# tingyu215/VACNIC

Hardware: AMD Instinct MI355X
Metric: train samples/sec, BART-large + CLIP ViT-L/14 full VACNIC step, GoodNews-shaped batch (higher is better)
Workload: dtype bf16

## Files before the change

### vacnic_amd/csrc/attn.hip

```cpp
#include "common.h"

namespace {

constexpr float FMIN = -3.4028234663852886e38f;
constexpr int OOB = 0x7ffffff0;
constexpr int TILE_B = 64 * 64 * 2;

__device__ __forceinline__ int swz(int row) { return (((row >> 1) & 1) << 2) | ((row >> 2) & 3); }

__device__ __forceinline__ void stage64(__amdgpu_buffer_rsrc_t rsrc, char* tile, int row0, int nrows, int ld,
                                        int wave, int lane) {
#pragma unroll
  for (int i = 0; i < 2; ++i) {
    const int blk = wave * 2 + i;
    const int row = blk * 8 + (lane >> 3);
    const int lc = (lane & 7) ^ swz(row);
    const int gr = row0 + row;
    const int voff = gr < nrows ? (int)(((unsigned)gr * (unsigned)ld + (unsigned)(lc * 8)) * 2u) : OOB;
    __builtin_amdgcn_raw_ptr_buffer_load_lds(rsrc, LDS_PTR(tile + blk * 1024), 16, voff, 0, 0, 0);
  }
}

__device__ __forceinline__ bf16x8 frag_row(const char* tile, int rbase, int ks, int lane) {
  const int row = rbase + (lane & 31);
  const int chunk = 2 * ks + (lane >> 5);
  return *(const bf16x8*)(tile + row * 128 + ((chunk ^ swz(row)) << 4));
}
__device__ __forceinline__ bf16x8 frag_tr(const char* tile, int rbase, int cbase, int lane) {
  const int g = lane >> 4, i = lane & 15, h = lane >> 5;
  const int col = cbase + 16 * (g & 1) + 4 * (i & 3);
  bf16x8 r;
#pragma unroll
  for (int hh = 0; hh < 2; ++hh) {
    const int row = rbase + 8 * hh + 4 * h + (i >> 2);
    const char* a = tile + row * 128 + (((col >> 3) ^ swz(row)) << 4) + (col & 7) * 2;
    bf16x4 t = __builtin_amdgcn_ds_read_tr16_b64_v4i16((__attribute__((address_space(3))) bf16x4*)LDS_PTR(a));
    r[4 * hh + 0] = t[0]; r[4 * hh + 1] = t[1]; r[4 * hh + 2] = t[2]; r[4 * hh + 3] = t[3];
  }
  return r;
}
__device__ __forceinline__ bf16x8 pack_acc(const f32x16& x, int s) {
  bf16x8 r;
#pragma unroll
  for (int j = 0; j < 8; ++j) r[j] = (short)f2bf(x[8 * s + j]);
  return r;
}
__device__ __forceinline__ bf16x8 gload8(__amdgpu_buffer_rsrc_t rsrc, int voff) {
  u32x4 v = __builtin_amdgcn_raw_buffer_load_b128(rsrc, voff, 0, 0);
  return *(bf16x8*)&v;
}
__device__ __forceinline__ int acc_row(int r, int h) { return (r & 3) + 8 * (r >> 2) + 4 * h; }

__device__ __forceinline__ void lds_barrier() {
  asm volatile("s_waitcnt lgkmcnt(0)" ::: "memory");
  __builtin_amdgcn_s_barrier();
}

struct AttnP {
  const bf16_t* q; const bf16_t* k; const bf16_t* v; bf16_t* out; float* lse;
  const bf16_t* dout; const float* delta; float* delta_out; bf16_t* dq; bf16_t* dk; bf16_t* dv;
  const uint8_t* key_mask;
  int B, H, Tq, Tk;
  int ldq, ldk, ldv, ldo, lddq, lddk, lddv;
  long bsq, bsk, bsv, bso, bsdq, bsdk, bsdv;
  int causal; float scale;
  unsigned drop_thr; float drop_inv; unsigned long long drop_seed; const unsigned long long* drop_seed_dev;
};

struct DropCtx { unsigned long long seed; unsigned long long bh_base; unsigned pk_per_row; unsigned thr; float inv; };

__device__ __forceinline__ DropCtx drop_ctx(const AttnP& p, int b, int hd) {
  DropCtx d;
  d.seed = p.drop_seed_dev ? p.drop_seed ^ (*p.drop_seed_dev * 0x9E3779B97F4A7C15ull) : p.drop_seed;
  d.pk_per_row = (unsigned)((p.Tk + 3) >> 2);
  d.bh_base = ((unsigned long long)b * p.H + hd) * (unsigned long long)((p.Tq + 3) >> 2) * d.pk_per_row;
  d.thr = p.drop_thr; d.inv = p.drop_inv;
  return d;
}
__device__ __forceinline__ void drop_patch(const DropCtx& d, int q, int k, uint32_t w[4]) {
  const unsigned long long idx = d.bh_base + (unsigned long long)(q >> 2) * d.pk_per_row + (unsigned)(k >> 2);
  philox4x32((uint32_t)idx, (uint32_t)(idx >> 32), 0x41545444u, 0u, (uint32_t)d.seed, (uint32_t)(d.seed >> 32), w);
}
#define VAC_QUAD_BCAST(V_, G_) ((uint32_t)__builtin_amdgcn_update_dpp(0, (int)(V_), (G_) * 0x55, 0xf, 0xf, true))
__device__ __forceinline__ void drop_block_keys(const DropCtx& d, int q, int kblock, int lane, uint32_t mw[4]) {
  const int i = lane & 3;
  uint32_t w[4];
  drop_patch(d, q, kblock + 8 * i, w);
#define VAC_TAKE(G_)                                                                                   \
  {                                                                                                    \
    const uint32_t t0 = VAC_QUAD_BCAST(w[0], G_), t1 = VAC_QUAD_BCAST(w[1], G_);                       \
    const uint32_t t2 = VAC_QUAD_BCAST(w[2], G_), t3 = VAC_QUAD_BCAST(w[3], G_);                       \
    mw[G_] = i == 0 ? t0 : i == 1 ? t1 : i == 2 ? t2 : t3;                                             \
  }
  VAC_TAKE(0) VAC_TAKE(1) VAC_TAKE(2) VAC_TAKE(3)
#undef VAC_TAKE
}
__device__ __forceinline__ void drop_word_factors(const DropCtx& d, uint32_t x, float m[4]) {
#pragma unroll
  for (int e = 0; e < 4; ++e) m[e] = ((x >> (8 * e)) & 0xffu) >= d.thr ? d.inv : 0.f;
}
__device__ __forceinline__ void drop_block_queries(const DropCtx& d, int qblock, int k, int lane, uint32_t mb[4]) {
  const int i = lane & 3, sh = 8 * i;
  uint32_t w[4];
  drop_patch(d, qblock + 8 * i, k, w);
#define VAC_TAKE(G_)                                                                                   \
  {                                                                                                    \
    const uint32_t t0 = VAC_QUAD_BCAST(w[0], G_), t1 = VAC_QUAD_BCAST(w[1], G_);                       \
    const uint32_t t2 = VAC_QUAD_BCAST(w[2], G_), t3 = VAC_QUAD_BCAST(w[3], G_);                       \
    mb[G_] = ((t0 >> sh) & 0xffu) | (((t1 >> sh) & 0xffu) << 8) | (((t2 >> sh) & 0xffu) << 16) | (((t3 >> sh) & 0xffu) << 24); \
  }
  VAC_TAKE(0) VAC_TAKE(1) VAC_TAKE(2) VAC_TAKE(3)
#undef VAC_TAKE
}

__device__ __forceinline__ __amdgpu_buffer_rsrc_t make_rsrc(const bf16_t* base, int rows, int ld) {
  const unsigned bytes = rows > 0 ? ((unsigned)(rows - 1) * (unsigned)ld + 64u) * 2u : 0u;
  return __builtin_amdgcn_make_buffer_rsrc((void*)base, 0, bytes, 0x00020000);
}

__device__ __forceinline__ void fill_key_bias(float* kbias, unsigned* dirty, const uint8_t* mask_row, int Tk, int Tk_pad) {
  for (int j = threadIdx.x; j < Tk_pad; j += 256) {
    float b = 0.f;
    if (j >= Tk) b = -INFINITY;
    else if (mask_row && mask_row[j] == 0) b = FMIN;
    kbias[j] = b;
    const unsigned long long any = __builtin_amdgcn_ballot_w64(b != 0.f);
    if ((threadIdx.x & 63) == 0) dirty[j >> 6] = any != 0ull;
  }
}


__device__ __forceinline__ void xcd_order(int nblk, int H, int nbh, int& blk, int& hd, int& b) {
  const int L = blockIdx.x;
  int bh;
  if ((nbh & 7) == 0) { const int x = L & 7, j = L >> 3; bh = x + 8 * (j / nblk); blk = j % nblk; }
  else { bh = L / nblk; blk = L % nblk; }
  b = bh / H; hd = bh - b * H;
}

template <bool CAUSAL, bool DROP>
__global__ __launch_bounds__(256, 2) void attn_fwd_kernel(AttnP p) {
  extern __shared__ __attribute__((aligned(16))) char smem[];
  const int tid = threadIdx.x, lane = tid & 63;
  const int wave = __builtin_amdgcn_readfirstlane(tid >> 6);
  int b, hd, qblk;
  xcd_order((p.Tq + 127) >> 7, p.H, p.B * p.H, qblk, hd, b);
  const int q0 = qblk * 128 + wave * 32;
  const int ql = lane & 31, hh = lane >> 5;
  const int Tk_pad = (p.Tk + 63) & ~63;
// ... 72 lines not shown
        }
      m_run = m_new;
    } else {
#pragma unroll
      for (int kb2 = 0; kb2 < 2; ++kb2) {
#pragma unroll
        for (int g = 0; g < 4; ++g) {
          const int kbase = t * 64 + kb2 * 32 + 8 * g + 4 * hh;
          const f32x4 bias = *(const f32x4*)(kbias + kbase);
#pragma unroll
          for (int e = 0; e < 4; ++e) {
            float v = fmaf(s[kb2][4 * g + e], scale2, bias[e]);
            if (CAUSAL && (kbase + e) > qidx) v += FMIN;
            s[kb2][4 * g + e] = v;
            tmax = fmaxf(tmax, v);
          }
        }
      }
      tmax = fmaxf(tmax, __shfl_xor(tmax, 32, 64));
      const float m_new = fmaxf(m_run, tmax);
      alpha = __builtin_amdgcn_exp2f(m_run - m_new);
#pragma unroll
      for (int kb2 = 0; kb2 < 2; ++kb2)
#pragma unroll
        for (int r = 0; r < 16; ++r) {
          const float e = __builtin_amdgcn_exp2f(s[kb2][r] - m_new);
          s[kb2][r] = e;
          psum += e;
        }
      m_run = m_new;
    }
    l_run = l_run * alpha + psum;
    if (DROP) {
#pragma unroll
      for (int kb2 = 0; kb2 < 2; ++kb2) {
        uint32_t mw[4];
        drop_block_keys(dctx, qidx, t * 64 + kb2 * 32 + 4 * hh, lane, mw);
#pragma unroll
        for (int g = 0; g < 4; ++g) {
          float mk[4];
          drop_word_factors(dctx, mw[g], mk);
#pragma unroll
          for (int e = 0; e < 4; ++e) s[kb2][4 * g + e] *= mk[e];
        }
      }
    }
#pragma unroll
    for (int r = 0; r < 16; ++r) { o[0][r] *= alpha; o[1][r] *= alpha; }
#pragma unroll
    for (int kb2 = 0; kb2 < 2; ++kb2)
#pragma unroll
      for (int ss = 0; ss < 2; ++ss) {
        const bf16x8 pf = pack_acc(s[kb2], ss);
#pragma unroll
        for (int hb = 0; hb < 2; ++hb)
          o[hb] = __builtin_amdgcn_mfma_f32_32x32x16_bf16(frag_tr(vt, kb2 * 32 + 16 * ss, hb * 32, lane), pf, o[hb], 0, 0, 0);
      }
    lds_barrier();
  }

  const float l_tot = l_run + __shfl_xor(l_run, 32, 64);
  const float inv = 1.f / l_tot;
  {
    char* ot = smem + wave * 4096;
#pragma unroll
    for (int hb = 0; hb < 2; ++hb)
#pragma unroll
      for (int g = 0; g < 4; ++g) {
        const u32x2 pk = {pack2bf(o[hb][4 * g] * inv, o[hb][4 * g + 1] * inv),
                          pack2bf(o[hb][4 * g + 2] * inv, o[hb][4 * g + 3] * inv)};
        const int c16 = hb * 4 + g;
        *(u32x2*)(ot + ql * 128 + ((c16 ^ (ql & 7)) << 4) + 8 * hh) = pk;
      }
    asm volatile("s_waitcnt lgkmcnt(0)" ::: "memory");
#pragma unroll
    for (int i = 0; i < 4; ++i) {
      const int row = (lane >> 3) + 8 * i, c16 = lane & 7;
      const int qrow = q0 + row;
      const u32x4 v = *(const u32x4*)(ot + row * 128 + ((c16 ^ (row & 7)) << 4));
      if (qrow < p.Tq) *(u32x4*)(p.out + (long)b * p.bso + (long)qrow * p.ldo + hd * 64 + c16 * 8) = v;
    }
  }
  if (qidx < p.Tq && p.lse && hh == 0) p.lse[((long)b * p.H + hd) * p.Tq + qidx] = m_run * 0.6931471805599453f + __logf(l_tot);
}

__global__ __launch_bounds__(256) void attn_delta_kernel(const bf16_t* __restrict__ o, const bf16_t* __restrict__ dout,
                                                         float* __restrict__ delta, int B, int H, int Tq, int ldo,
                                                         long bso) {
  const int lane = threadIdx.x & 63;
  const long row = (long)blockIdx.x * 4 + (threadIdx.x >> 6);
  if (row >= (long)B * Tq) return;
  const int b = (int)(row / Tq), q = (int)(row % Tq);
  const bf16_t* orow = o + (long)b * bso + (long)q * ldo;
  const bf16_t* drow = dout + (long)b * bso + (long)q * ldo;
  for (int c = lane; c < H * 8; c += 64) {
    u32x4 a = *(const u32x4*)(orow + c * 8), d = *(const u32x4*)(drow + c * 8);
    float s = 0.f;
#pragma unroll
    for (int i = 0; i < 4; ++i) {
      s += __uint_as_float(a[i] << 16) * __uint_as_float(d[i] << 16);
      s += __uint_as_float(a[i] & 0xffff0000u) * __uint_as_float(d[i] & 0xffff0000u);
    }
    s += __shfl_xor(s, 1, 64); s += __shfl_xor(s, 2, 64); s += __shfl_xor(s, 4, 64);
    if ((c & 7) == 0) delta[((long)b * H + (c >> 3)) * Tq + q] = s;
  }
}

template <bool DROP>
__global__ __launch_bounds__(256, 2) void attn_bwd_dkv_kernel(AttnP p) {
  extern __shared__ __attribute__((aligned(16))) char smem[];
  const int tid = threadIdx.x, lane = tid & 63;
  const int wave = __builtin_amdgcn_readfirstlane(tid >> 6);
  int b, hd, kblk;
  xcd_order((p.Tk + 127) >> 7, p.H, p.B * p.H, kblk, hd, b);
  const int k0 = kblk * 128 + wave * 32;
  const int kl = lane & 31, hh = lane >> 5;
  const int kidx = k0 + kl;
  float* stats = (float*)(smem + 4 * TILE_B);
  constexpr float LOG2E = 1.4426950408889634f;
  const float scale2 = p.scale * LOG2E;

  const bf16_t* qb = p.q + (long)b * p.bsq + hd * 64;
  const bf16_t* kb = p.k + (long)b * p.bsk + hd * 64;
  const bf16_t* vb = p.v + (long)b * p.bsv + hd * 64;
  const bf16_t* dob = p.dout + (long)b * p.bso + hd * 64;
  __amdgpu_buffer_rsrc_t qs = make_rsrc(qb, p.Tq, p.ldq);
  __amdgpu_buffer_rsrc_t ks = make_rsrc(kb, p.Tk, p.ldk);
  __amdgpu_buffer_rsrc_t vs = make_rsrc(vb, p.Tk, p.ldv);
  __amdgpu_buffer_rsrc_t dos = make_rsrc(dob, p.Tq, p.ldo);
  const float* lse = p.lse + ((long)b * p.H + hd) * p.Tq;
  const float* delta = p.delta + ((long)b * p.H + hd) * p.Tq;

  const int nq_tiles = (p.Tq + 63) >> 6;
  int t_begin = 0;
  if (p.causal) t_begin = min(nq_tiles, (kblk * 128) >> 6);

  bf16x8 kf[4], vf[4];
#pragma unroll
  for (int s = 0; s < 4; ++s) {
    kf[s] = gload8(ks, kidx < p.Tk ? (int)(((unsigned)kidx * (unsigned)p.ldk + 16u * s + 8u * hh) * 2u) : OOB);
    vf[s] = gload8(vs, kidx < p.Tk ? (int)(((unsigned)kidx * (unsigned)p.ldv + 16u * s + 8u * hh) * 2u) : OOB);
  }
  float kbias = 0.f;
  if (kidx >= p.Tk) kbias = -INFINITY;
  else if (p.key_mask && p.key_mask[(long)b * p.Tk + kidx] == 0) kbias = FMIN;

  f32x16 dk[2], dv[2];
  dk[0] = (f32x16)(0.f); dk[1] = (f32x16)(0.f); dv[0] = (f32x16)(0.f); dv[1] = (f32x16)(0.f);
  DropCtx dctx;
  if (DROP) dctx = drop_ctx(p, b, hd);

  auto load_stat = [&](int t) -> float {
    float v = 0.f;
    if (tid < 128) {
      const int qi = t * 64 + (tid & 63);
      if (tid < 64) v = qi < p.Tq ? lse[qi] : INFINITY;
      else v = qi < p.Tq ? delta[qi] : 0.f;
    }
    return v;
  };
  auto put_stat = [&](float* st, float sv) {
    if (tid < 128) st[tid] = sv;
    if (tid < 64) st[128 + tid] = -sv * LOG2E;
  };
  const bool plain = !p.causal && __builtin_amdgcn_ballot_w64(kbias != 0.f) == 0ull;

  if (t_begin < nq_tiles) {
    const float sv = load_stat(t_begin);
    stage64(qs, smem, t_begin * 64, p.Tq, p.ldq, wave, lane);
    stage64(dos, smem + TILE_B, t_begin * 64, p.Tq, p.ldo, wave, lane);
    put_stat(stats, sv);
  }
  for (int t = t_begin; t < nq_tiles; ++t) {
    const int cur = (t - t_begin) & 1;
    char* qt = smem + cur * (2 * TILE_B);
    char* dot = qt + TILE_B;
    if (t + 1 < nq_tiles) {
      char* nq = smem + (cur ^ 1) * (2 * TILE_B);
      const float sv = load_stat(t + 1);
      stage64(qs, nq, (t + 1) * 64, p.Tq, p.ldq, wave, lane);
      stage64(dos, nq + TILE_B, (t + 1) * 64, p.Tq, p.ldo, wave, lane);
      put_stat(stats + (cur ^ 1) * 192, sv);
      asm volatile("s_waitcnt vmcnt(4)" ::: "memory");
    } else {
      asm volatile("s_waitcnt vmcnt(0)" ::: "memory");
    }
    lds_barrier();
    const float* st = stats + cur * 192;

#pragma unroll
    for (int qb2 = 0; qb2 < 2; ++qb2) {
      f32x16 s = (f32x16)(0.f), dp = (f32x16)(0.f);
#pragma unroll
      for (int ks4 = 0; ks4 < 4; ++ks4) {
        s = __builtin_amdgcn_mfma_f32_32x32x16_bf16(frag_row(qt, qb2 * 32, ks4, lane), kf[ks4], s, 0, 0, 0);
        dp = __builtin_amdgcn_mfma_f32_32x32x16_bf16(frag_row(dot, qb2 * 32, ks4, lane), vf[ks4], dp, 0, 0, 0);
      }
      uint32_t mb[4];
      if (DROP) drop_block_queries(dctx, t * 64 + qb2 * 32 + 4 * hh, kidx, lane, mb);
#pragma unroll
      for (int g = 0; g < 4; ++g) {
        const int ql0 = qb2 * 32 + 8 * g + 4 * hh;
        const f32x4 l4 = *(const f32x4*)(st + ql0);
        const f32x4 d4 = *(const f32x4*)(st + 64 + ql0);
        float mq[4] = {1.f, 1.f, 1.f, 1.f};
        if (DROP) drop_word_factors(dctx, mb[g], mq);
        if (plain) {
          const f32x4 nl4 = *(const f32x4*)(st + 128 + ql0);
#pragma unroll
          for (int e = 0; e < 4; ++e) {
            const float pe = __builtin_amdgcn_exp2f(fmaf(s[4 * g + e], scale2, nl4[e]));
            s[4 * g + e] = DROP ? pe * mq[e] : pe;
            dp[4 * g + e] = pe * ((DROP ? dp[4 * g + e] * mq[e] : dp[4 * g + e]) - d4[e]);
          }
        } else {
#pragma unroll
          for (int e = 0; e < 4; ++e) {
            float v = s[4 * g + e] * p.scale + kbias;
            if (p.causal && kidx > (t * 64 + ql0 + e)) v += FMIN;
            const float pe = __expf(v - l4[e]);
            s[4 * g + e] = DROP ? pe * mq[e] : pe;
            dp[4 * g + e] = pe * ((DROP ? dp[4 * g + e] * mq[e] : dp[4 * g + e]) - d4[e]);
          }
        }
      }
#pragma unroll
      for (int ss = 0; ss < 2; ++ss) {
        const bf16x8 pf = pack_acc(s, ss), dsf = pack_acc(dp, ss);
#pragma unroll
        for (int hb = 0; hb < 2; ++hb) {
          dv[hb] = __builtin_amdgcn_mfma_f32_32x32x16_bf16(frag_tr(dot, qb2 * 32 + 16 * ss, hb * 32, lane), pf, dv[hb], 0, 0, 0);
          dk[hb] = __builtin_amdgcn_mfma_f32_32x32x16_bf16(frag_tr(qt, qb2 * 32 + 16 * ss, hb * 32, lane), dsf, dk[hb], 0, 0, 0);
        }
      }
    }
    lds_barrier();
  }

  if (kidx < p.Tk) {
    bf16_t* dkrow = p.dk + (long)b * p.bsdk + (long)kidx * p.lddk + hd * 64;
    bf16_t* dvrow = p.dv + (long)b * p.bsdv + (long)kidx * p.lddv + hd * 64;
#pragma unroll
    for (int hb = 0; hb < 2; ++hb)
#pragma unroll
      for (int g = 0; g < 4; ++g) {
        u32x2 a = {pack2bf(dk[hb][4 * g] * p.scale, dk[hb][4 * g + 1] * p.scale), pack2bf(dk[hb][4 * g + 2] * p.scale, dk[hb][4 * g + 3] * p.scale)};
        u32x2 c = {pack2bf(dv[hb][4 * g], dv[hb][4 * g + 1]), pack2bf(dv[hb][4 * g + 2], dv[hb][4 * g + 3])};
        *(u32x2*)(dkrow + hb * 32 + 8 * g + 4 * hh) = a;
        *(u32x2*)(dvrow + hb * 32 + 8 * g + 4 * hh) = c;
      }
  }
}

template <bool DROP, bool DELTA_PASS>
__global__ __launch_bounds__(256, 2) void attn_bwd_dq_kernel(AttnP p) {
  extern __shared__ __attribute__((aligned(16))) char smem[];
  const int tid = threadIdx.x, lane = tid & 63;
  const int wave = __builtin_amdgcn_readfirstlane(tid >> 6);
  int b, hd, qblk;
  xcd_order((p.Tq + 127) >> 7, p.H, p.B * p.H, qblk, hd, b);
  const int q0 = qblk * 128 + wave * 32;
  const int ql = lane & 31, hh = lane >> 5;
  const int qidx = q0 + ql;
  const int Tk_pad = (p.Tk + 63) & ~63;
  float* kbias = (float*)(smem + 4 * TILE_B);
  unsigned* dirty = (unsigned*)(kbias + Tk_pad);
  constexpr float LOG2E = 1.4426950408889634f;
  const float scale2 = p.scale * LOG2E;

  const bf16_t* qb = p.q + (long)b * p.bsq + hd * 64;
  const bf16_t* kb = p.k + (long)b * p.bsk + hd * 64;
  const bf16_t* vb = p.v + (long)b * p.bsv + hd * 64;
  const bf16_t* dob = p.dout + (long)b * p.bso + hd * 64;
  __amdgpu_buffer_rsrc_t qs = make_rsrc(qb, p.Tq, p.ldq);
  __amdgpu_buffer_rsrc_t ks = make_rsrc(kb, p.Tk, p.ldk);
  __amdgpu_buffer_rsrc_t vs = make_rsrc(vb, p.Tk, p.ldv);
  __amdgpu_buffer_rsrc_t dos = make_rsrc(dob, p.Tq, p.ldo);

  int ntile = Tk_pad >> 6;
  if (p.causal) ntile = min(ntile, (min(p.Tq, qblk * 128 + 128) + 63) >> 6);

  stage64(ks, smem, 0, p.Tk, p.ldk, wave, lane);
  stage64(vs, smem + TILE_B, 0, p.Tk, p.ldv, wave, lane);
  fill_key_bias(kbias, dirty, p.key_mask ? p.key_mask + (long)b * p.Tk : nullptr, p.Tk, Tk_pad);

  bf16x8 qf[4], dof[4];
#pragma unroll
  for (int s = 0; s < 4; ++s) {
    qf[s] = gload8(qs, qidx < p.Tq ? (int)(((unsigned)qidx * (unsigned)p.ldq + 16u * s + 8u * hh) * 2u) : OOB);
    dof[s] = gload8(dos, qidx < p.Tq ? (int)(((unsigned)qidx * (unsigned)p.ldo + 16u * s + 8u * hh) * 2u) : OOB);
  }
  float lse_q = INFINITY, delta_q = 0.f;
  if (qidx < p.Tq) {
    lse_q = p.lse[((long)b * p.H + hd) * p.Tq + qidx];
    if (!DELTA_PASS) delta_q = p.delta[((long)b * p.H + hd) * p.Tq + qidx];
  }
  const float nl2 = -lse_q * LOG2E;
  float dsum = 0.f;
  f32x16 dq[2];
  dq[0] = (f32x16)(0.f); dq[1] = (f32x16)(0.f);
  DropCtx dctx;
  if (DROP) dctx = drop_ctx(p, b, hd);

  for (int t = 0; t < ntile; ++t) {
    const int cur = t & 1;
    char* kt = smem + cur * (2 * TILE_B);
    char* vt = kt + TILE_B;
    if (t + 1 < ntile) {
      char* nk = smem + (cur ^ 1) * (2 * TILE_B);
      stage64(ks, nk, (t + 1) * 64, p.Tk, p.ldk, wave, lane);
      stage64(vs, nk + TILE_B, (t + 1) * 64, p.Tk, p.ldv, wave, lane);
      asm volatile("s_waitcnt vmcnt(4)" ::: "memory");
    } else {
      asm volatile("s_waitcnt vmcnt(0)" ::: "memory");
    }
    lds_barrier();
    const bool plain = !p.causal && __builtin_amdgcn_readfirstlane((int)dirty[t]) == 0;
#pragma unroll
    for (int kb2 = 0; kb2 < 2; ++kb2) {
      f32x16 s = (f32x16)(0.f), dp = (f32x16)(0.f);
#pragma unroll
      for (int ks4 = 0; ks4 < 4; ++ks4) {
        s = __builtin_amdgcn_mfma_f32_32x32x16_bf16(frag_row(kt, kb2 * 32, ks4, lane), qf[ks4], s, 0, 0, 0);
        dp = __builtin_amdgcn_mfma_f32_32x32x16_bf16(frag_row(vt, kb2 * 32, ks4, lane), dof[ks4], dp, 0, 0, 0);
      }
      uint32_t mw[4];
      if (DROP) drop_block_keys(dctx, qidx, t * 64 + kb2 * 32 + 4 * hh, lane, mw);
#pragma unroll
      for (int g = 0; g < 4; ++g) {
        const int kbase = t * 64 + kb2 * 32 + 8 * g + 4 * hh;
        float mk[4] = {1.f, 1.f, 1.f, 1.f};
        if (DROP) drop_word_factors(dctx, mw[g], mk);
        if (plain) {
#pragma unroll
          for (int e = 0; e < 4; ++e) {
            const float pe = __builtin_amdgcn_exp2f(fmaf(s[4 * g + e], scale2, nl2));
            const float dpm = DROP ? dp[4 * g + e] * mk[e] : dp[4 * g + e];
            if (DELTA_PASS) dsum += pe * dpm;
            else dp[4 * g + e] = pe * (dpm - delta_q);
          }
        } else {
          const f32x4 bias = *(const f32x4*)(kbias + kbase);
#pragma unroll
          for (int e = 0; e < 4; ++e) {
            float v = s[4 * g + e] * p.scale + bias[e];
            if (p.causal && (kbase + e) > qidx) v += FMIN;
            const float pe = __expf(v - lse_q);
            const float dpm = DROP ? dp[4 * g + e] * mk[e] : dp[4 * g + e];
            if (DELTA_PASS) dsum += pe * dpm;
            else dp[4 * g + e] = pe * (dpm - delta_q);
          }
        }
      }
      if (!DELTA_PASS) {
#pragma unroll
        for (int ss = 0; ss < 2; ++ss) {
          const bf16x8 dsf = pack_acc(dp, ss);
#pragma unroll
          for (int hb = 0; hb < 2; ++hb)
            dq[hb] = __builtin_amdgcn_mfma_f32_32x32x16_bf16(frag_tr(kt, kb2 * 32 + 16 * ss, hb * 32, lane), dsf, dq[hb], 0, 0, 0);
        }
      }
    }
    lds_barrier();
  }
  if (DELTA_PASS) {
    dsum += __shfl_xor(dsum, 32, 64);
    if (qidx < p.Tq && hh == 0) p.delta_out[((long)b * p.H + hd) * p.Tq + qidx] = dsum;
    return;
  }
  if (qidx < p.Tq) {
    bf16_t* drow = p.dq + (long)b * p.bsdq + (long)qidx * p.lddq + hd * 64;
#pragma unroll
    for (int hb = 0; hb < 2; ++hb)
#pragma unroll
      for (int g = 0; g < 4; ++g) {
        u32x2 a = {pack2bf(dq[hb][4 * g] * p.scale, dq[hb][4 * g + 1] * p.scale), pack2bf(dq[hb][4 * g + 2] * p.scale, dq[hb][4 * g + 3] * p.scale)};
        *(u32x2*)(drow + hb * 32 + 8 * g + 4 * hh) = a;
      }
  }
}

int set_dropout(AttnP& p, float p_drop, uint64_t seed, const uint64_t* seed_dev, const char* who) {
  if (!(p_drop >= 0.f && p_drop < 1.f)) { vacnic_set_error("%s: p_drop must be in [0, 1)", who); return VACNIC_BAD_SHAPE; }
  unsigned thr = (unsigned)(p_drop * 256.f + 0.5f);
  if (thr > 255) thr = 255;
  p.drop_thr = thr;
  p.drop_inv = 256.f / (256.f - (float)thr);
  p.drop_seed = seed; p.drop_seed_dev = (const unsigned long long*)seed_dev;
  return VACNIC_OK;
}

int check_common(int64_t B, int64_t H, int64_t Tq, int64_t Tk, int64_t ldq, int64_t ldk, int64_t ldv, int64_t ldo,
                 const char* who) {
  if (B <= 0 || H <= 0 || Tq <= 0 || Tk <= 0) {
    vacnic_set_error("%s: empty problem B=%ld H=%ld Tq=%ld Tk=%ld", who, (long)B, (long)H, (long)Tq, (long)Tk);
    return VACNIC_BAD_SHAPE;
  }
  if ((ldq & 7) || (ldk & 7) || (ldv & 7) || (ldo & 7)) {
    vacnic_set_error("%s: row strides must be multiples of 8 elements", who);
    return VACNIC_MISALIGNED;
  }
  if (Tk > 8192 || H > 65535 || B > 65535) {
    vacnic_set_error("%s: Tk=%ld / H / B beyond supported range", who, (long)Tk);
    return VACNIC_UNSUPPORTED;
  }
  return VACNIC_OK;
}

}


template <int NWV>
__global__ __launch_bounds__(64 * NWV) void attn_decode_kernel(AttnP p) {
  extern __shared__ float probs[];
  const int lane = threadIdx.x & 63, h = blockIdx.x, b = blockIdx.y;
  const int wv = NWV == 1 ? 0 : __builtin_amdgcn_readfirstlane(threadIdx.x >> 6);
  const int per = (p.Tk + NWV - 1) / NWV;
  const int k_lo = wv * per, k_hi = min(p.Tk, k_lo + per);
  const bf16_t* q = p.q + (long)b * p.bsq + h * 64;
  const bf16_t* kb = p.k + (long)b * p.bsk + h * 64;
  const bf16_t* vb = p.v + (long)b * p.bsv + h * 64;
  const uint8_t* km = p.key_mask ? p.key_mask + (long)b * p.Tk : nullptr;
  float qf[64];
#pragma unroll
  for (int c = 0; c < 8; ++c) {
    const u32x4 r = *(const u32x4*)(q + c * 8);
#pragma unroll
    for (int i = 0; i < 4; ++i) { qf[c * 8 + 2 * i] = __uint_as_float(r[i] << 16); qf[c * 8 + 2 * i + 1] = __uint_as_float(r[i] & 0xffff0000u); }
  }
  float m = -INFINITY;
  for (int key0 = k_lo + lane; key0 < k_hi; key0 += 256) {
    u32x4 kr[4][8];
#pragma unroll
    for (int u = 0; u < 4; ++u) {
      const int key = key0 + 64 * u;
      const bf16_t* krow = kb + (long)(key < k_hi ? key : key0) * p.ldk;
#pragma unroll
      for (int c = 0; c < 8; ++c) kr[u][c] = *(const u32x4*)(krow + c * 8);
    }
#pragma unroll
    for (int u = 0; u < 4; ++u) {
      const int key = key0 + 64 * u;
      if (key < k_hi) {
        float dot = 0.f;
#pragma unroll
        for (int c = 0; c < 8; ++c)
#pragma unroll
          for (int i = 0; i < 4; ++i) {
            dot += qf[c * 8 + 2 * i] * __uint_as_float(kr[u][c][i] << 16);
            dot += qf[c * 8 + 2 * i + 1] * __uint_as_float(kr[u][c][i] & 0xffff0000u);
          }
        float sc = dot * p.scale;
        if (km && km[key] == 0) sc += -3.4028234663852886e38f;
        probs[key] = sc;
        m = fmaxf(m, sc);
      }
    }
  }
  m = wave_max(m);
  float l = 0.f;
  for (int key = k_lo + lane; key < k_hi; key += 64) {
// ... 38 lines not shown
    }
    if (lane == 0) { pm[wv] = m; pl[wv] = l; }
    __syncthreads();
    if (wv != 0) return;
    float gm = pm[0];
#pragma unroll
    for (int w = 1; w < NWV; ++w) gm = fmaxf(gm, pm[w]);
    float gl = 0.f;
#pragma unroll
    for (int j = 0; j < 8; ++j) acc[j] = 0.f;
#pragma unroll
    for (int w = 0; w < NWV; ++w) {
      const float sc = pl[w] > 0.f ? __expf(pm[w] - gm) : 0.f;
      gl += pl[w] * sc;
      if (kg == 0) {
#pragma unroll
        for (int j = 0; j < 8; ++j) acc[j] += pacc[w * 64 + dc * 8 + j] * sc;
      }
    }
    m = gm; l = gl;
  }
  if (kg == 0) {
    const float inv = 1.f / l;
    bf16_t* o = p.out + (long)b * p.bso + h * 64 + dc * 8;
    *(u32x4*)o = (u32x4){pack2bf(acc[0] * inv, acc[1] * inv), pack2bf(acc[2] * inv, acc[3] * inv),
                         pack2bf(acc[4] * inv, acc[5] * inv), pack2bf(acc[6] * inv, acc[7] * inv)};
  }
  if (p.lse && lane == 0) p.lse[((long)b * p.H + h)] = m + logf(l);
}

extern "C" int vacnic_attn_fwd(const vacnic_attn_fwd_args* a, void* stream) {
  VPLAN_REC_STRUCT(vacnic_attn_fwd, a, stream);
  VCHECK(a && a->q && a->k && a->v && a->out, VACNIC_BAD_SHAPE, "attn_fwd: null operand");
  if (int e = check_common(a->B, a->H, a->Tq, a->Tk, a->ldq, a->ldk, a->ldv, a->ldo, "attn_fwd")) return e;
  VCHECK(aligned16(a->q) && aligned16(a->k) && aligned16(a->v) && aligned16(a->out) && !(a->bsq & 7) && !(a->bsk & 7) &&
         !(a->bsv & 7) && !(a->bso & 7), VACNIC_MISALIGNED, "attn_fwd: pointers/batch strides must be 16-byte aligned");
  AttnP p = {};
  p.q = (const bf16_t*)a->q; p.k = (const bf16_t*)a->k; p.v = (const bf16_t*)a->v; p.out = (bf16_t*)a->out;
  p.lse = a->lse; p.key_mask = a->key_mask;
  p.B = (int)a->B; p.H = (int)a->H; p.Tq = (int)a->Tq; p.Tk = (int)a->Tk;
  p.ldq = (int)a->ldq; p.ldk = (int)a->ldk; p.ldv = (int)a->ldv; p.ldo = (int)a->ldo;
  p.bsq = a->bsq; p.bsk = a->bsk; p.bsv = a->bsv; p.bso = a->bso;
  p.causal = a->causal; p.scale = a->scale;
  if (int e = set_dropout(p, a->p_drop, a->seed, a->seed_dev, "attn_fwd")) return e;
  if (p.Tq == 1 && !p.causal && p.Tk <= 16384 && !p.drop_thr) {
    if (p.Tk >= 256) hipLaunchKernelGGL(attn_decode_kernel<4>, dim3(p.H, p.B), dim3(256), (size_t)(p.Tk + 4 * 64 + 8) * 4, (hipStream_t)stream, p);
    else hipLaunchKernelGGL(attn_decode_kernel<1>, dim3(p.H, p.B), dim3(64), (size_t)p.Tk * 4, (hipStream_t)stream, p);
    VLAUNCH_CHECK();
    return VACNIC_OK;
  }
  const int Tk_pad = (p.Tk + 63) & ~63;
  dim3 grid((unsigned)(((p.Tq + 127) / 128) * p.H * p.B));
  const size_t lds = 4 * TILE_B + Tk_pad * 4 + (Tk_pad >> 6) * 4;
  hipStream_t st = (hipStream_t)stream;
  if (p.drop_thr) {
    if (p.causal) hipLaunchKernelGGL((attn_fwd_kernel<true, true>), grid, dim3(256), lds, st, p);
    else hipLaunchKernelGGL((attn_fwd_kernel<false, true>), grid, dim3(256), lds, st, p);
  } else {
    if (p.causal) hipLaunchKernelGGL((attn_fwd_kernel<true, false>), grid, dim3(256), lds, st, p);
    else hipLaunchKernelGGL((attn_fwd_kernel<false, false>), grid, dim3(256), lds, st, p);
  }
  VLAUNCH_CHECK();
  return VACNIC_OK;
}

extern "C" int vacnic_attn_bwd(const vacnic_attn_bwd_args* a, void* stream) {
  VPLAN_REC_STRUCT(vacnic_attn_bwd, a, stream);
  VCHECK(a && a->q && a->k && a->v && a->out && a->dout && a->lse && a->delta && a->dq && a->dk && a->dv,
         VACNIC_BAD_SHAPE, "attn_bwd: null operand");
  if (int e = check_common(a->B, a->H, a->Tq, a->Tk, a->ldq, a->ldk, a->ldv, a->ldo, "attn_bwd")) return e;
  VCHECK(!(a->lddq & 7) && !(a->lddk & 7) && !(a->lddv & 7) && !(a->bsq & 7) && !(a->bsk & 7) && !(a->bsv & 7) &&
         !(a->bso & 7) && !(a->bsdq & 7) && !(a->bsdk & 7) && !(a->bsdv & 7), VACNIC_MISALIGNED,
         "attn_bwd: strides must be multiples of 8 elements");
  AttnP p = {};
  p.q = (const bf16_t*)a->q; p.k = (const bf16_t*)a->k; p.v = (const bf16_t*)a->v;
  p.dout = (const bf16_t*)a->dout; p.lse = (float*)a->lse; p.delta = a->delta;
  p.dq = (bf16_t*)a->dq; p.dk = (bf16_t*)a->dk; p.dv = (bf16_t*)a->dv; p.key_mask = a->key_mask;
  p.B = (int)a->B; p.H = (int)a->H; p.Tq = (int)a->Tq; p.Tk = (int)a->Tk;
  p.ldq = (int)a->ldq; p.ldk = (int)a->ldk; p.ldv = (int)a->ldv; p.ldo = (int)a->ldo;
  p.lddq = (int)a->lddq; p.lddk = (int)a->lddk; p.lddv = (int)a->lddv;
  p.bsq = a->bsq; p.bsk = a->bsk; p.bsv = a->bsv; p.bso = a->bso;
  p.bsdq = a->bsdq; p.bsdk = a->bsdk; p.bsdv = a->bsdv;
  p.causal = a->causal; p.scale = a->scale;
  if (int e = set_dropout(p, a->p_drop, a->seed, a->seed_dev, "attn_bwd")) return e;
  hipStream_t s = (hipStream_t)stream;
  const long rows = (long)p.B * p.Tq;
  const int Tk_pad = (p.Tk + 63) & ~63;
  const dim3 gkv((unsigned)(((p.Tk + 127) / 128) * p.H * p.B)), gq((unsigned)(((p.Tq + 127) / 128) * p.H * p.B));
  const size_t lds_q = 4 * TILE_B + Tk_pad * 4 + (Tk_pad >> 6) * 4;
  p.delta_out = a->delta;
  if (p.Tq <= 128) {
    if (p.drop_thr) hipLaunchKernelGGL((attn_bwd_dq_kernel<true, true>), gq, dim3(256), lds_q, s, p);
    else hipLaunchKernelGGL((attn_bwd_dq_kernel<false, true>), gq, dim3(256), lds_q, s, p);
  } else {
    hipLaunchKernelGGL(attn_delta_kernel, dim3((unsigned)((rows + 3) / 4)), dim3(256), 0, s, (const bf16_t*)a->out,
                       (const bf16_t*)a->dout, a->delta, p.B, p.H, p.Tq, p.ldo, (long)p.bso);
  }
  VLAUNCH_CHECK();
  if (p.drop_thr) hipLaunchKernelGGL(attn_bwd_dkv_kernel<true>, gkv, dim3(256), 4 * TILE_B + 2 * 192 * 4, s, p);
  else hipLaunchKernelGGL(attn_bwd_dkv_kernel<false>, gkv, dim3(256), 4 * TILE_B + 2 * 192 * 4, s, p);
  VLAUNCH_CHECK();
  if (p.drop_thr) hipLaunchKernelGGL((attn_bwd_dq_kernel<true, false>), gq, dim3(256), lds_q, s, p);
  else hipLaunchKernelGGL((attn_bwd_dq_kernel<false, false>), gq, dim3(256), lds_q, s, p);
  VLAUNCH_CHECK();
  return VACNIC_OK;
}

struct ProbsP {
  const bf16_t* q; const bf16_t* k; float* out; const uint8_t* key_mask;
  int B, H, Tq, Tk, ldq, ldk;
  long bsq, bsk;
  int causal; float scale;
};

constexpr int PROBS_WAVE_B = 32 * 64 * 4;

__device__ __forceinline__ void probs_load_k(__amdgpu_buffer_rsrc_t ks, int t, int Tk, int ldk, int tid, u32x4 kr[2]) {
#pragma unroll
  for (int i = 0; i < 2; ++i) {
    const int row = i * 32 + (tid >> 3), gr = t * 64 + row;
    kr[i] = __builtin_amdgcn_raw_buffer_load_b128(ks, gr < Tk ? (int)(((unsigned)gr * (unsigned)ldk + (unsigned)((tid & 7) * 8)) * 2u) : OOB, 0, 0);
  }
}
__device__ __forceinline__ void probs_put_k(char* tile, int tid, const u32x4 kr[2]) {
#pragma unroll
  for (int i = 0; i < 2; ++i) {
    const int row = i * 32 + (tid >> 3);
    *(u32x4*)(tile + row * 128 + (((tid & 7) ^ swz(row)) << 4)) = kr[i];
  }
}

template <bool CAUSAL>
__device__ __forceinline__ void probs_scores(const char* kt, const bf16x8 qf[4], const float* kbias, int t, int lane,
                                             int qidx, float scale2, f32x16 s[2]) {
  const int hh = lane >> 5;
#pragma unroll
  for (int kb2 = 0; kb2 < 2; ++kb2) {
    s[kb2] = (f32x16)(0.f);
#pragma unroll
    for (int ks4 = 0; ks4 < 4; ++ks4)
      s[kb2] = __builtin_amdgcn_mfma_f32_32x32x16_bf16(frag_row(kt, kb2 * 32, ks4, lane), qf[ks4], s[kb2], 0, 0, 0);
#pragma unroll
    for (int g = 0; g < 4; ++g) {
      const int kbase = t * 64 + kb2 * 32 + 8 * g + 4 * hh;
      const f32x4 bias = *(const f32x4*)(kbias + kbase);
#pragma unroll
      for (int e = 0; e < 4; ++e) {
        float v = fmaf(s[kb2][4 * g + e], scale2, bias[e]);
        if (CAUSAL && (kbase + e) > qidx) v += FMIN;
        s[kb2][4 * g + e] = v;
      }
    }
  }
}

template <bool CAUSAL, bool VEC>
__global__ __launch_bounds__(256, 2) void attn_probs_kernel(ProbsP p) {
  extern __shared__ __attribute__((aligned(16))) char smem[];
  const int tid = threadIdx.x, lane = tid & 63;
  const int wave = __builtin_amdgcn_readfirstlane(tid >> 6);
  int b, hd, qblk;
  xcd_order((p.Tq + 127) >> 7, p.H, p.B * p.H, qblk, hd, b);
  const int q0 = qblk * 128 + wave * 32;
  const int ql = lane & 31, hh = lane >> 5;
  const int Tk_pad = (p.Tk + 63) & ~63;
  char* ot = smem + wave * PROBS_WAVE_B;
  char* kring = smem + 4 * PROBS_WAVE_B;
  float* kbias = (float*)(kring + 2 * TILE_B);

  __amdgpu_buffer_rsrc_t qs = make_rsrc(p.q + (long)b * p.bsq + hd * 64, p.Tq, p.ldq);
  __amdgpu_buffer_rsrc_t ks = make_rsrc(p.k + (long)b * p.bsk + hd * 64, p.Tk, p.ldk);
  float* ob = p.out + ((long)b * p.H + hd) * ((long)p.Tq * p.Tk);
  __amdgpu_buffer_rsrc_t os = __builtin_amdgcn_make_buffer_rsrc((void*)ob, 0, (unsigned)p.Tq * (unsigned)p.Tk * 4u, 0x00020000);
// ... 121 lines not shown
```

Baseline: 507.5.

## Fuse attention backward into one kernel for short query lengths

Adds a single-kernel attention backward path for Tq<=64 that computes delta, dK/dV and dQ in one workgroup per (batch, head), replacing three kernel launches. Q and dO stay resident in LDS, dS is kept in LDS so dQ can be accumulated in the same pass, and K/V tiles are double-buffered. It also adds an LDS-staged path that writes dQ/dK/dV as coalesced 16-byte rows when the output pointers are 16-byte aligned. The cost is much higher LDS use per block and less grid parallelism, since there is one block per head.

```diff
diff --git a/vacnic_amd/csrc/attn.hip b/vacnic_amd/csrc/attn.hip
--- a/vacnic_amd/csrc/attn.hip
+++ b/vacnic_amd/csrc/attn.hip
@@ -65,6 +65,7 @@
   long bsq, bsk, bsv, bso, bsdq, bsdk, bsdv;
   int causal; float scale;
   unsigned drop_thr; float drop_inv; unsigned long long drop_seed; const unsigned long long* drop_seed_dev;
+  int rows16;
 };
 
 struct DropCtx { unsigned long long seed; unsigned long long bh_base; unsigned pk_per_row; unsigned thr; float inv; };
@@ -303,6 +304,27 @@
     }
   }
   if (qidx < p.Tq && p.lse && hh == 0) p.lse[((long)b * p.H + hd) * p.Tq + qidx] = m_run * 0.6931471805599453f + __logf(l_tot);
+}
+
+__device__ __forceinline__ void store_rows32(char* ot, const f32x16 (&x)[2], float scale, bf16_t* dst, int ld, int row0, int nrows,
+                                             int lane) {
+  const int rl = lane & 31, hh = lane >> 5;
+#pragma unroll
+  for (int hb = 0; hb < 2; ++hb)
+#pragma unroll
+    for (int g = 0; g < 4; ++g) {
+      const u32x2 pk = {pack2bf(x[hb][4 * g] * scale, x[hb][4 * g + 1] * scale),
+                        pack2bf(x[hb][4 * g + 2] * scale, x[hb][4 * g + 3] * scale)};
+      const int c16 = hb * 4 + g;
+      *(u32x2*)(ot + rl * 128 + ((c16 ^ (rl & 7)) << 4) + 8 * hh) = pk;
+    }
+  asm volatile("s_waitcnt lgkmcnt(0)" ::: "memory");
+#pragma unroll
+  for (int i = 0; i < 4; ++i) {
+    const int row = (lane >> 3) + 8 * i, c16 = lane & 7;
+    const u32x4 v = *(const u32x4*)(ot + row * 128 + ((c16 ^ (row & 7)) << 4));
+    if (row0 + row < nrows) *(u32x4*)(dst + (long)row * ld + c16 * 8) = v;
+  }
 }
 
 __global__ __launch_bounds__(256) void attn_delta_kernel(const bf16_t* __restrict__ o, const bf16_t* __restrict__ dout,
@@ -458,7 +480,13 @@
     lds_barrier();
   }
 
-  if (kidx < p.Tk) {
+  if (p.rows16) {
+    if (k0 < p.Tk) {
+      char* ot = smem + wave * 8192;
+      store_rows32(ot, dk, p.scale, p.dk + (long)b * p.bsdk + (long)k0 * p.lddk + hd * 64, p.lddk, k0, p.Tk, lane);
+      store_rows32(ot + 4096, dv, 1.f, p.dv + (long)b * p.bsdv + (long)k0 * p.lddv + hd * 64, p.lddv, k0, p.Tk, lane);
+    }
+  } else if (kidx < p.Tk) {
     bf16_t* dkrow = p.dk + (long)b * p.bsdk + (long)kidx * p.lddk + hd * 64;
     bf16_t* dvrow = p.dv + (long)b * p.bsdv + (long)kidx * p.lddv + hd * 64;
 #pragma unroll
@@ -590,7 +618,10 @@
     if (qidx < p.Tq && hh == 0) p.delta_out[((long)b * p.H + hd) * p.Tq + qidx] = dsum;
     return;
   }
-  if (qidx < p.Tq) {
+  if (p.rows16) {
+    if (q0 < p.Tq)
+      store_rows32(smem + wave * 4096, dq, p.scale, p.dq + (long)b * p.bsdq + (long)q0 * p.lddq + hd * 64, p.lddq, q0, p.Tq, lane);
+  } else if (qidx < p.Tq) {
     bf16_t* drow = p.dq + (long)b * p.bsdq + (long)qidx * p.lddq + hd * 64;
 #pragma unroll
     for (int hb = 0; hb < 2; ++hb)
@@ -599,6 +630,301 @@
         u32x2 a = {pack2bf(dq[hb][4 * g] * p.scale, dq[hb][4 * g + 1] * p.scale), pack2bf(dq[hb][4 * g + 2] * p.scale, dq[hb][4 * g + 3] * p.scale)};
         *(u32x2*)(drow + hb * 32 + 8 * g + 4 * hh) = a;
       }
+  }
+}
+
+constexpr int SHORT_LDS = 8 * TILE_B + (256 + 128 + 128 + 8) * 4;
+
+template <bool DROP>
+__global__ __launch_bounds__(256, 2) void attn_bwd_short_kernel(AttnP p) {
+  extern __shared__ __attribute__((aligned(16))) char smem[];
+  const int tid = threadIdx.x, lane = tid & 63;
+  const int wave = __builtin_amdgcn_readfirstlane(tid >> 6);
+  const int b = blockIdx.x / p.H, hd = blockIdx.x - b * p.H;
+  const int rl = lane & 31, hh = lane >> 5;
+  const int qb = wave & 1, wh = wave >> 1;
+  const int nqb = p.Tq > 32 ? 2 : 1;
+  char* qt = smem;
+  char* dot = smem + TILE_B;
+  char* ring = smem + 2 * TILE_B;
+  char* dst = smem + 6 * TILE_B;
+  float* stats = (float*)(smem + 8 * TILE_B);
+  float* part = stats + 256;
+  float* tbias = part + 128;
+  unsigned* dirty = (unsigned*)(tbias + 128);
+  unsigned* anyvalid = dirty + 2;
+  constexpr float LOG2E = 1.4426950408889634f;
+  const float scale2 = p.scale * LOG2E;
+
+  const bf16_t* vb = p.v + (long)b * p.bsv + hd * 64;
+  __amdgpu_buffer_rsrc_t qs = make_rsrc(p.q + (long)b * p.bsq + hd * 64, p.Tq, p.ldq);
+  __amdgpu_buffer_rsrc_t ks = make_rsrc(p.k + (long)b * p.bsk + hd * 64, p.Tk, p.ldk);
+  __amdgpu_buffer_rsrc_t vs = make_rsrc(vb, p.Tk, p.ldv);
+  __amdgpu_buffer_rsrc_t dos = make_rsrc(p.dout + (long)b * p.bso + hd * 64, p.Tq, p.ldo);
+  const uint8_t* mrow = p.key_mask ? p.key_mask + (long)b * p.Tk : nullptr;
+  auto key_bias = [&](int key) -> float {
+    float v = 0.f;
+    if (key >= p.Tk) v = -INFINITY;
+    else if (mrow && mrow[key] == 0) v = FMIN;
+    return v;
+  };
+  auto put_bias = [&](int slot, float v) {
+    if (wave == 0) {
+      tbias[slot * 64 + lane] = v;
+      const unsigned long long any = __builtin_amdgcn_ballot_w64(v != 0.f);
+      if (lane == 0) dirty[slot] = any != 0ull;
+    }
+  };
+  DropCtx dctx;
+  if (DROP) dctx = drop_ctx(p, b, hd);
+
+  int ntile = (p.Tk + 63) >> 6;
+  if (p.causal) ntile = min(ntile, (p.Tq + 63) >> 6);
+  {
+    float b0 = 0.f, l0 = INFINITY;
+    bool valid = mrow == nullptr;
+    if (mrow)
+      for (int j = tid; j < p.Tk; j += 256) valid |= mrow[j] != 0;
+    if (wave == 0) {
+      b0 = key_bias(lane);
+      if (lane < p.Tq) l0 = p.lse[((long)b * p.H + hd) * p.Tq + lane];
+    }
+    stage64(qs, qt, 0, p.Tq, p.ldq, wave, lane);
+    stage64(dos, dot, 0, p.Tq, p.ldo, wave, lane);
+    stage64(ks, ring, 0, p.Tk, p.ldk, wave, lane);
+    stage64(vs, ring + TILE_B, 0, p.Tk, p.ldv, wave, lane);
+    if (wave == 0) {
+      stats[lane] = l0; stats[128 + lane] = -l0 * LOG2E;
+      stats[192 + lane] = lane < p.Tq ? 1.f / (float)(p.causal ? min(lane, p.Tk - 1) + 1 : p.Tk) : 0.f;
+    }
+    {
+      const unsigned long long any = __builtin_amdgcn_ballot_w64(valid);
+      if (lane == 0) anyvalid[wave] = any != 0ull;
+    }
+    put_bias(0, b0);
+    asm volatile("s_waitcnt vmcnt(0)" ::: "memory");
+    lds_barrier();
+  }
+  const int qidx = qb * 32 + rl;
+  float dsum = 0.f;
+  const bool allmasked = __builtin_amdgcn_readfirstlane((int)(anyvalid[0] | anyvalid[1] | anyvalid[2] | anyvalid[3])) == 0;
+  {
+    bf16x8 qf[4], dof[4];
+#pragma unroll
+    for (int s = 0; s < 4; ++s) { qf[s] = frag_row(qt, qb * 32, s, lane); dof[s] = frag_row(dot, qb * 32, s, lane); }
+    const float lse_q = stats[qidx], nl2 = stats[128 + qidx], uni_q = stats[192 + qidx];
+    for (int t = 0; t < ntile; ++t) {
+      const int cur = t & 1;
+      char* kt = ring + cur * (2 * TILE_B);
+      char* vt = kt + TILE_B;
+      float bn = 0.f;
+      if (t + 1 < ntile) {
+        char* nk = ring + (cur ^ 1) * (2 * TILE_B);
+        if (wave == 0) bn = key_bias((t + 1) * 64 + lane);
+        stage64(ks, nk, (t + 1) * 64, p.Tk, p.ldk, wave, lane);
+        stage64(vs, nk + TILE_B, (t + 1) * 64, p.Tk, p.ldv, wave, lane);
+        asm volatile("s_waitcnt vmcnt(4)" ::: "memory");
+      } else {
+        asm volatile("s_waitcnt vmcnt(0)" ::: "memory");
+      }
+      lds_barrier();
+      const bool plain = !p.causal && __builtin_amdgcn_readfirstlane((int)dirty[cur]) == 0;
+      if (qb < nqb) {
+        f32x16 s = (f32x16)(0.f), dp = (f32x16)(0.f);
+#pragma unroll
+        for (int ks4 = 0; ks4 < 4; ++ks4) {
+          s = __builtin_amdgcn_mfma_f32_32x32x16_bf16(frag_row(kt, wh * 32, ks4, lane), qf[ks4], s, 0, 0, 0);
+          dp = __builtin_amdgcn_mfma_f32_32x32x16_bf16(frag_row(vt, wh * 32, ks4, lane), dof[ks4], dp, 0, 0, 0);
+        }
+        uint32_t mw[4];
+        if (DROP) drop_block_keys(dctx, qidx, t * 64 + wh * 32 + 4 * hh, lane, mw);
+#pragma unroll
+        for (int g = 0; g < 4; ++g) {
+          const int kl0 = wh * 32 + 8 * g + 4 * hh;
+          float mk[4] = {1.f, 1.f, 1.f, 1.f};
+          if (DROP) drop_word_factors(dctx, mw[g], mk);
+          if (plain) {
+#pragma unroll
+            for (int e = 0; e < 4; ++e) {
+              const float pe = __builtin_amdgcn_exp2f(fmaf(s[4 * g + e], scale2, nl2));
+              dsum += pe * (DROP ? dp[4 * g + e] * mk[e] : dp[4 * g + e]);
+            }
+          } else if (allmasked) {
+            const f32x4 bias = *(const f32x4*)(tbias + cur * 64 + kl0);
+#pragma unroll
+            for (int e = 0; e < 4; ++e) {
+              const float pe = (bias[e] == FMIN && !(p.causal && (t * 64 + kl0 + e) > qidx)) ? uni_q : 0.f;
+              dsum += pe * (DROP ? dp[4 * g + e] * mk[e] : dp[4 * g + e]);
+            }
+          } else {
+            const f32x4 bias = *(const f32x4*)(tbias + cur * 64 + kl0);
+#pragma unroll
+            for (int e = 0; e < 4; ++e) {
+              float v = s[4 * g + e] * p.scale + bias[e];
+              if (p.causal && (t * 64 + kl0 + e) > qidx) v += FMIN;
+              const float pe = __expf(v - lse_q);
+              dsum += pe * (DROP ? dp[4 * g + e] * mk[e] : dp[4 * g + e]);
+            }
+          }
+        }
+      }
+      if (t + 1 < ntile) put_bias(cur ^ 1, bn);
+      lds_barrier();
+    }
+  }
+
+  const int ntile2 = (p.Tk + 127) >> 7;
+  char* ktile = ring;
+  char* vtile = ring + 2 * TILE_B;
+  float kbias = key_bias(wave * 32 + rl);
+  stage64(ks, ktile, 0, p.Tk, p.ldk, wave, lane);
+  stage64(ks, ktile + TILE_B, 64, p.Tk, p.ldk, wave, lane);
+  stage64(vs, vtile, 0, p.Tk, p.ldv, wave, lane);
+  stage64(vs, vtile + TILE_B, 64, p.Tk, p.ldv, wave, lane);
+  dsum += __shfl_xor(dsum, 32, 64);
+  if (hh == 0) part[wh * 64 + qidx] = dsum;
+  lds_barrier();
+  if (wave == 0) {
+    const float d = part[lane] + part[64 + lane];
+    stats[64 + lane] = d;
+    if (lane < p.Tq) p.delta_out[((long)b * p.H + hd) * p.Tq + lane] = d;
+  }
+
+  f32x16 dq = (f32x16)(0.f);
+  for (int t = 0; t < ntile2; ++t) {
+    asm volatile("s_waitcnt vmcnt(0)" ::: "memory");
+    lds_barrier();
+    int la = lane, lb = lane;
+    asm volatile("" : "+v"(la));
+    const int rl = la & 31, hh = la >> 5;
+    const int k0 = t * 128 + wave * 32, kidx = k0 + rl;
+    const bool plain = !p.causal && __builtin_amdgcn_ballot_w64(kbias != 0.f) == 0ull;
+    f32x16 dk[2], dv[2];
+    dk[0] = (f32x16)(0.f); dk[1] = (f32x16)(0.f); dv[0] = (f32x16)(0.f); dv[1] = (f32x16)(0.f);
+    {
+#pragma unroll
+      for (int qb2 = 0; qb2 < 2; ++qb2) {
+        if (qb2 < nqb) {
+          bf16x8 kf[4], vf[4];
+#pragma unroll
+          for (int s = 0; s < 4; ++s) { kf[s] = frag_row(ktile, wave * 32, s, la); vf[s] = frag_row(vtile, wave * 32, s, la); }
+          f32x16 s = (f32x16)(0.f), dp = (f32x16)(0.f);
+#pragma unroll
+          for (int ks4 = 0; ks4 < 4; ++ks4) {
+            s = __builtin_amdgcn_mfma_f32_32x32x16_bf16(frag_row(qt, qb2 * 32, ks4, la), kf[ks4], s, 0, 0, 0);
+            dp = __builtin_amdgcn_mfma_f32_32x32x16_bf16(frag_row(dot, qb2 * 32, ks4, la), vf[ks4], dp, 0, 0, 0);
+          }
+          uint32_t mb[4];
+          if (DROP) drop_block_queries(dctx, qb2 * 32 + 4 * hh, kidx, lane, mb);
+#pragma unroll
+          for (int g = 0; g < 4; ++g) {
+            const int ql0 = qb2 * 32 + 8 * g + 4 * hh;
+            const f32x4 l4 = *(const f32x4*)(stats + ql0);
+            const f32x4 d4 = *(const f32x4*)(stats + 64 + ql0);
+            float mq[4] = {1.f, 1.f, 1.f, 1.f};
+            if (DROP) drop_word_factors(dctx, mb[g], mq);
+            if (plain) {
+              const f32x4 nl4 = *(const f32x4*)(stats + 128 + ql0);
+#pragma unroll
+              for (int e = 0; e < 4; ++e) {
+                const float pe = __builtin_amdgcn_exp2f(fmaf(s[4 * g + e], scale2, nl4[e]));
+                s[4 * g + e] = DROP ? pe * mq[e] : pe;
+                dp[4 * g + e] = pe * ((DROP ? dp[4 * g + e] * mq[e] : dp[4 * g + e]) - d4[e]);
+              }
+            } else if (allmasked) {
+              const f32x4 u4 = *(const f32x4*)(stats + 192 + ql0);
+#pragma unroll
+              for (int e = 0; e < 4; ++e) {
+                const float pe = (kbias == FMIN && !(p.causal && kidx > (ql0 + e))) ? u4[e] : 0.f;
+                s[4 * g + e] = DROP ? pe * mq[e] : pe;
+                dp[4 * g + e] = pe * ((DROP ? dp[4 * g + e] * mq[e] : dp[4 * g + e]) - d4[e]);
+              }
+            } else {
+#pragma unroll
+              for (int e = 0; e < 4; ++e) {
+                float v = s[4 * g + e] * p.scale + kbias;
+                if (p.causal && kidx > (ql0 + e)) v += FMIN;
+                const float pe = __expf(v - l4[e]);
+                s[4 * g + e] = DROP ? pe * mq[e] : pe;
+                dp[4 * g + e] = pe * ((DROP ? dp[4 * g + e] * mq[e] : dp[4 * g + e]) - d4[e]);
+              }
+            }
+            const int row = wave * 32 + rl;
+            const u32x2 pk = {pack2bf(dp[4 * g], dp[4 * g + 1]), pack2bf(dp[4 * g + 2], dp[4 * g + 3])};
+            *(u32x2*)(dst + row * 128 + (((qb2 * 4 + g) ^ swz(row)) << 4) + 8 * hh) = pk;
+          }
+#pragma unroll
+          for (int ss = 0; ss < 2; ++ss) {
+            const bf16x8 pf = pack_acc(s, ss), dsf = pack_acc(dp, ss);
+#pragma unroll
+            for (int hb = 0; hb < 2; ++hb) {
+              dv[hb] = __builtin_amdgcn_mfma_f32_32x32x16_bf16(frag_tr(dot, qb2 * 32 + 16 * ss, hb * 32, la), pf, dv[hb], 0, 0, 0);
+              dk[hb] = __builtin_amdgcn_mfma_f32_32x32x16_bf16(frag_tr(qt, qb2 * 32 + 16 * ss, hb * 32, la), dsf, dk[hb], 0, 0, 0);
+            }
+          }
+        }
+      }
+    }
+    lds_barrier();
+    if (t + 1 < ntile2) {
+      kbias = key_bias(kidx + 128);
+      stage64(vs, vtile, (t + 1) * 128, p.Tk, p.ldv, wave, lane);
+      stage64(vs, vtile + TILE_B, (t + 1) * 128 + 64, p.Tk, p.ldv, wave, lane);
+    }
+    asm volatile("" : "+v"(lb));
+    if (qb < nqb) {
+#pragma unroll
+      for (int k16 = 0; k16 < 8; ++k16)
+        dq = __builtin_amdgcn_mfma_f32_32x32x16_bf16(frag_tr(ktile, 16 * k16, wh * 32, lb), frag_tr(dst, 16 * k16, qb * 32, lb), dq, 0, 0, 0);
+    }
+    lds_barrier();
+    if (t + 1 < ntile2) {
+      stage64(ks, ktile, (t + 1) * 128, p.Tk, p.ldk, wave, lane);
+      stage64(ks, ktile + TILE_B, (t + 1) * 128 + 64, p.Tk, p.ldk, wave, lane);
+    }
+    if (p.rows16) {
+      if (k0 < p.Tk) {
+        char* ot = dst + wave * 4096;
+        store_rows32(ot, dk, p.scale, p.dk + (long)b * p.bsdk + (long)k0 * p.lddk + hd * 64, p.lddk, k0, p.Tk, lb);
+        store_rows32(ot, dv, 1.f, p.dv + (long)b * p.bsdv + (long)k0 * p.lddv + hd * 64, p.lddv, k0, p.Tk, lb);
+      }
+    } else if (kidx < p.Tk) {
+      bf16_t* dkrow = p.dk + (long)b * p.bsdk + (long)kidx * p.lddk + hd * 64;
+      bf16_t* dvrow = p.dv + (long)b * p.bsdv + (long)kidx * p.lddv + hd * 64;
+#pragma unroll
+      for (int hb = 0; hb < 2; ++hb)
+#pragma unroll
+        for (int g = 0; g < 4; ++g) {
+          u32x2 a = {pack2bf(dk[hb][4 * g] * p.scale, dk[hb][4 * g + 1] * p.scale), pack2bf(dk[hb][4 * g + 2] * p.scale, dk[hb][4 * g + 3] * p.scale)};
+          u32x2 c = {pack2bf(dv[hb][4 * g], dv[hb][4 * g + 1]), pack2bf(dv[hb][4 * g + 2], dv[hb][4 * g + 3])};
+          *(u32x2*)(dkrow + hb * 32 + 8 * g + 4 * hh) = a;
+          *(u32x2*)(dvrow + hb * 32 + 8 * g + 4 * hh) = c;
+        }
+    }
+  }
+
+  lds_barrier();
+  int le = lane;
+  asm volatile("" : "+v"(le));
+  if (qb < nqb) {
+    char* ot = dst + qb * 4096;
+    const int rl = le & 31, hh = le >> 5;
+#pragma unroll
+    for (int g = 0; g < 4; ++g) {
+      const u32x2 pk = {pack2bf(dq[4 * g] * p.scale, dq[4 * g + 1] * p.scale), pack2bf(dq[4 * g + 2] * p.scale, dq[4 * g + 3] * p.scale)};
+      *(u32x2*)(ot + rl * 128 + (((wh * 4 + g) ^ (rl & 7)) << 4) + 8 * hh) = pk;
+    }
+  }
+  lds_barrier();
+#pragma unroll
+  for (int i = 0; i < 2; ++i) {
+    const int r = wave * 8 + (le >> 3), c16 = le & 7, row = i * 32 + r;
+    if (row < p.Tq) {
+      const u32x4 v = *(const u32x4*)(dst + i * 4096 + r * 128 + ((c16 ^ (r & 7)) << 4));
+      bf16_t* d = p.dq + (long)b * p.bsdq + (long)row * p.lddq + hd * 64 + c16 * 8;
+      if (p.rows16) *(u32x4*)d = v;
+      else { *(u32x2*)d = (u32x2){v[0], v[1]}; *(u32x2*)(d + 4) = (u32x2){v[2], v[3]}; }
+    }
   }
 }
 
@@ -803,6 +1129,7 @@
   p.bsq = a->bsq; p.bsk = a->bsk; p.bsv = a->bsv; p.bso = a->bso;
   p.bsdq = a->bsdq; p.bsdk = a->bsdk; p.bsdv = a->bsdv;
   p.causal = a->causal; p.scale = a->scale;
+  p.rows16 = aligned16(a->dq) && aligned16(a->dk) && aligned16(a->dv);
   if (int e = set_dropout(p, a->p_drop, a->seed, a->seed_dev, "attn_bwd")) return e;
   hipStream_t s = (hipStream_t)stream;
   const long rows = (long)p.B * p.Tq;
@@ -810,6 +1137,19 @@
   const dim3 gkv((unsigned)(((p.Tk + 127) / 128) * p.H * p.B)), gq((unsigned)(((p.Tq + 127) / 128) * p.H * p.B));
   const size_t lds_q = 4 * TILE_B + Tk_pad * 4 + (Tk_pad >> 6) * 4;
   p.delta_out = a->delta;
+  if (p.Tq <= 64) {
+    static bool once = false;
+    if (!once) {
+      (void)hipFuncSetAttribute((const void*)attn_bwd_short_kernel<true>, hipFuncAttributeMaxDynamicSharedMemorySize, SHORT_LDS);
+      (void)hipFuncSetAttribute((const void*)attn_bwd_short_kernel<false>, hipFuncAttributeMaxDynamicSharedMemorySize, SHORT_LDS);
+      once = true;
+    }
+    const dim3 gbh((unsigned)(p.H * p.B));
+    if (p.drop_thr) hipLaunchKernelGGL(attn_bwd_short_kernel<true>, gbh, dim3(256), SHORT_LDS, s, p);
+    else hipLaunchKernelGGL(attn_bwd_short_kernel<false>, gbh, dim3(256), SHORT_LDS, s, p);
+    VLAUNCH_CHECK();
+    return VACNIC_OK;
+  }
   if (p.Tq <= 128) {
     if (p.drop_thr) hipLaunchKernelGGL((attn_bwd_dq_kernel<true, true>), gq, dim3(256), lds_q, s, p);
     else hipLaunchKernelGGL((attn_bwd_dq_kernel<false, true>), gq, dim3(256), lds_q, s, p);
```

After: 514.9 (median of 6 runs). 1.5% higher.
